# exoplanet-dev/exoplanet

Hardware: AMD Instinct MI355X
Metric: light-curve evals/sec (value+grad) at 150k cadences (higher is better)
Workload: dtype f64; 1 GPU; BASELINE configs[1] (C2): single planet e=0.3 Kepler solve + quadratic limb-darkened transit, 150000 cadences, value+grad, use_in_transit=False: dense flux output; n_cadences=150000, draws_per_gpu=1024, global_draws=1024, parallelism=draws sharded over 1 GPU(s); one collective of per-draw scalars per step

## Files before the change

### exoplanet_amd/_lib.py

```python
import ctypes
import os

_HERE = os.path.dirname(os.path.abspath(__file__))
LIB_PATH = os.environ.get("EXOPLANET_AMD_LIB") or os.path.join(_HERE, "lib", "libexoplanet_amd.so")
ABI_VERSION = 21

_c_dp = ctypes.c_void_p
_i64 = ctypes.c_int64
_i32 = ctypes.c_int32
_u32 = ctypes.c_uint32

_SIGNATURES = {
    "exo_abi_version": (_i32, []),
    "exo_kepler_f64": (ctypes.c_int, [_c_dp, _c_dp, _c_dp, _c_dp, _i64, _c_dp]),
    "exo_selftest_orbit_pos_f32": (ctypes.c_int, [_c_dp, _c_dp, _c_dp, _c_dp, _i64, _c_dp]),
    "exo_quad_solution_vector_f64": (ctypes.c_int, [_c_dp, _c_dp, _c_dp, _c_dp, _c_dp, _i64, _c_dp]),
    "exo_contact_points_f64": (ctypes.c_int, [_c_dp] * 10 + [_i64, _c_dp]),
    "exo_transit_flux_fwd_f64": (
        ctypes.c_int,
        [_c_dp, _i64, _c_dp, _i64, _c_dp, _c_dp, _i32, _c_dp, _c_dp, _i64, _i32, _u32, _c_dp, _c_dp, _i64, _c_dp],
    ),
    "exo_transit_flux_fwd_ev_f64": (
        ctypes.c_int,
        [_c_dp, _i64, _c_dp, _i64, _c_dp, _c_dp, _i32, _c_dp, _c_dp, _i64, _i32, _u32, _c_dp, _c_dp, _i64, _c_dp,
         _c_dp, _c_dp],
    ),
    "exo_transit_flux_workspace_bytes": (_i64, [_i64, _i64, _i32]),
    "exo_transit_flux_sparse_layout": (ctypes.c_int, [_i64, _i64, _i32, ctypes.POINTER(_i64)]),
    "exo_transit_flux_vjp_f64": (
        ctypes.c_int,
        [_c_dp, _i64, _c_dp, _i64, _c_dp, _c_dp, _i32, _c_dp, _c_dp, _i64, _i32, _u32,
         _c_dp, _c_dp, _c_dp, _c_dp, _c_dp, _c_dp, _i64, _c_dp],
    ),
    "exo_transit_flux_vjp_ev_f64": (
        ctypes.c_int,
        [_c_dp, _i64, _c_dp, _i64, _c_dp, _c_dp, _i32, _c_dp, _c_dp, _i64, _i32, _u32,
         _c_dp, _c_dp, _c_dp, _c_dp, _c_dp, _c_dp, _i64, _c_dp, _c_dp, _c_dp],
    ),
    "exo_transit_flux_ttv_fwd_f64": (
        ctypes.c_int,
        [_c_dp, _i64, _c_dp, _i64, _c_dp, _c_dp, _i32, _c_dp, _c_dp, _i64, _i32, _u32, _c_dp, _c_dp, _i32,
         _c_dp, _c_dp, _i64, _c_dp],
    ),
# ... 192 lines not shown
```

### exoplanet_amd/csrc/exo_transit.hip

```cpp
#include <hip/hip_runtime.h>
#include <stdint.h>

#include "../../include/exoplanet_amd.h"
#include "exo_contact.hpp"
#include "exo_math.hpp"
#include "exo_pack_core.hpp"
#include "exo_transit_list.hpp"
#include "exo_transit_merge.hpp"
#include "exo_transit_runs.hpp"
#include "exo_transit_sample.hpp"
#include "exo_transit_window.hpp"

namespace {

inline int launch_status() { return hipGetLastError() == hipSuccess ? EXO_OK : EXO_ERR_LAUNCH; }

struct Chi2Args {
  const double* obs;
  const double* ivar;
  int64_t n_ivar;
  double* chi2;
  const NoiseIn* nz = nullptr;
};

// ... 42 lines not shown
constexpr uint32_t kLikelihoodRefuses = EXO_FLAG_PER_PLANET | EXO_FLAG_SPARSE | EXO_FLAG_EXACT_SCAN;
constexpr uint32_t kTimedLikelihoodRefuses = kLikelihoodRefuses | EXO_FLAG_SECONDARY | EXO_FLAG_LIGHT_DELAY;
constexpr uint32_t kJacRefuses = EXO_FLAG_PER_PLANET | EXO_FLAG_EXACT_SCAN | EXO_FLAG_LIGHT_DELAY;
inline bool layout_ok(const Sweep& s) { return !((s.flags & EXO_FLAG_CADENCE_MAJOR) && (s.flags & EXO_FLAG_PER_PLANET)); }
inline bool exposure_ok(const Sweep& s) { return s.n_texp <= 0 || (s.texp && s.stencil_dt && s.stencil_w); }
inline bool ttv_ok(const Ttv& v, bool reverse) {
  return v.edges && v.shift && v.n_edge >= 1 && v.n_edge <= EXO_MAX_TTV_EDGES && (!reverse || v.gshift);
}
inline bool grad_ptrs_ok(const Sweep& s, const SweepOut& o) {
  return s.params && s.ld && o.gparams && o.gld && (s.n_cad <= 0 || s.t);
}
inline bool runs_path(const Sweep& s) {
  if (s.has_ttv() && (s.flags & (EXO_FLAG_SECONDARY | EXO_FLAG_LIGHT_DELAY))) return false;
  return s.n_texp <= 1 && !(s.flags & EXO_FLAG_EXACT_SCAN);
}
inline bool grad_slots_fit(const Sweep& s) { return s.n_planet * kNG + 7 <= kBlock; }
inline bool fit_runs(const void* workspace, int64_t workspace_bytes, int64_t n_cad, int64_t n_draw, int32_t n_planet, RunWs* rw) {
  *rw = carve_runs(const_cast<void*>(workspace), n_cad, n_draw, n_planet);
  return workspace && workspace_bytes >= rw->bytes;
}
inline bool fit_runs(const Sweep& s, RunWs* rw) { return fit_runs(s.workspace, s.workspace_bytes, s.n_cad, s.n_draw, s.n_planet, rw); }
inline int zero_grads(const Sweep& s, const SweepOut& o) {
  if (!exo::zero_fill_async(o.gparams, (int64_t)(s.n_draw * s.n_planet * EXO_NPAR), s.st)) return EXO_ERR_LAUNCH;
  if (o.flux_dot && !exo::zero_fill_async(o.flux_dot, (int64_t)(s.n_draw), s.st)) return EXO_ERR_LAUNCH;
  return exo::zero_fill_async(o.gld, (int64_t)(s.n_draw * (s.secondary() ? 6 : 3)), s.st) ? EXO_OK : EXO_ERR_LAUNCH;
}
inline bool zero_gshift(const Sweep& s) {
  return exo::zero_fill_async(s.ttv.gshift, (int64_t)(s.n_draw * s.n_planet * (s.ttv.n_edge + 1)), s.st);
}

template <bool G, bool SEC, bool LDELAY = false, bool CHI2 = false, bool TTV = false, bool JAC = false>
inline void launch_runs(const Sweep& s, const RunWs& w, const double* gflux, const double* gsparse, double* vals, int32_t* vcad,
                        double* fill, double* partial, const FinishArgs& fin, int64_t chi2_nw = 0) {
  hipLaunchKernelGGL((transit_runs_kernel<G, SEC, LDELAY, CHI2, TTV, JAC>), dim3((unsigned)w.hb, (unsigned)s.n_draw), dim3(kBlock), 0,
                     s.st, s.t, s.n_cad, s.texp, s.n_texp, s.stencil_dt, s.stencil_w, (int)s.n_sub, s.params, s.ld, (int)s.n_planet,
                     s.flags, s.n_ev(), w.rl, gflux, gsparse, vals, vcad, fill, partial, chi2_nw, s.ttv, fin);
}
template <bool G>
inline void launch_runs_plain(const Sweep& s, const RunWs& w, const double* gflux, const double* gsparse, double* vals,
                              int32_t* vcad, double* fill, double* partial, const FinishArgs& fin) {
  exo::with_flag(s.secondary(), [&](auto sec) {
    exo::with_flag(s.flags & EXO_FLAG_LIGHT_DELAY, [&](auto ldl) {
      launch_runs<G, decltype(sec)::value, decltype(ldl)::value>(s, w, gflux, gsparse, vals, vcad, fill, partial, fin);
    });
  });
}
inline int enumerate_runs(const Sweep& s, const SweepOut& o, const RunWs& w) {
  const bool fused = (s.flags & EXO_FLAG_SORTED_TIMES) && !s.has_ttv();
  if (o.pack && (!fused || o.reuse_runs)) return EXO_ERR_INVALID_ARGUMENT;
  const int n_ev = s.n_ev();
  const dim3 lists((unsigned)(s.n_draw * s.n_planet * n_ev)), wave(64);
// ... 39 lines not shown
                       s.n_cad, s.flags, s.n_ev(), w.rl, w.vcad, f.chi2_part, f.n_chi2_part, f.chi2, f.ttv, o.chi2->nz->out);
  else
    hipLaunchKernelGGL(transit_finish_kernel, grid, block, 0, s.st, f.partial, w.hb, (int)s.n_planet, s.secondary(), o.gparams, o.gld,
                       f.dot, s.n_cad, s.flags, s.n_ev(), w.rl, f.vals, w.vcad, f.fill, f.chi2_part, f.n_chi2_part, f.chi2, f.ttv);
  return launch_status();
}

inline bool single_pass(const Sweep& s) { return s.n_planet == 1 && !s.secondary() && s.n_sub == 1; }
inline int likelihood_single_pass(const Sweep& s, const SweepOut& o, const RunWs& w) {
  const Chi2Args& c = *o.chi2;
  const bool fold = own_block_finishes(s, o, w), ldelay = s.flags & EXO_FLAG_LIGHT_DELAY;
  const FinishArgs fin{o.gparams, o.gld, c.chi2, fold ? 1 : 0, w.done};
  const auto launch = [&](auto ldl, auto tv) {
    constexpr bool LDELAY = decltype(ldl)::value, TTV = decltype(tv)::value;
    if (c.nz)
      hipLaunchKernelGGL((transit_runs_kernel<true, false, LDELAY, true, TTV, false, true>), dim3((unsigned)w.hb, (unsigned)s.n_draw),
                         dim3(kBlock), 0, s.st, s.t, s.n_cad, s.texp, s.n_texp, s.stencil_dt, s.stencil_w, (int)s.n_sub, s.params, s.ld,
                         (int)s.n_planet, s.flags, s.n_ev(), w.rl, c.obs, c.ivar, nullptr, nullptr, nullptr, w.partial, c.n_ivar,
                         s.ttv, fin, *c.nz);
    else
      launch_runs<true, false, LDELAY, true, TTV>(s, w, c.obs, c.ivar, nullptr, nullptr, nullptr, w.partial, fin, c.n_ivar);
  };
  if (s.has_ttv()) launch(std::false_type{}, std::true_type{});
  else if (ldelay) launch(std::true_type{}, std::false_type{});
  else launch(std::false_type{}, std::false_type{});
  if (launch_status() != EXO_OK) return EXO_ERR_LAUNCH;
  if (fold) return EXO_OK;
  return launch_finish(s, o, w, FinishIn{w.partial, c.chi2, nullptr, nullptr, nullptr, 0, nullptr, s.ttv});
}

inline int likelihood_three_sweeps(const Sweep& s, const SweepOut& o, const RunWs& w) {
  const Chi2Args& c = *o.chi2;
  const FinishArgs no_fin{nullptr, nullptr, nullptr, 0, nullptr};
  const dim3 grid(kResidualBlocks, (unsigned)s.n_draw), block(kBlock);
// ... 56 lines not shown

int64_t exo_transit_flux_workspace_bytes(int64_t n_cad, int64_t n_draw, int32_t n_planet) {
  if (n_cad < 0 || n_draw < 0 || n_planet < 1) return -1;
  if (n_cad == 0 || n_draw == 0) return 0;
  int bpd, tpb;
  transit_geometry(n_cad, n_draw, &bpd, &tpb);
  const Workspace w = carve(nullptr, n_draw, bpd, tpb, n_planet);
  const RunWs r = carve_runs(nullptr, n_cad, n_draw, n_planet);
  return w.bytes > r.bytes ? w.bytes : r.bytes;
}

int exo_transit_flux_sparse_layout(int64_t n_cad, int64_t n_draw, int32_t n_planet, int64_t* out) {
  if (n_cad < 0 || n_draw < 0 || n_planet < 1 || !out) return EXO_ERR_INVALID_ARGUMENT;
  const RunWs r = carve_runs(nullptr, n_cad, n_draw, n_planet);
  out[0] = r.off_nrun; out[1] = r.off_runs; out[2] = r.off_pre_all; out[3] = r.off_vals; out[4] = r.rl.r_max;
  return EXO_OK;
}

int exo_transit_sparse_scatter_f64(const void* workspace, int64_t workspace_bytes, int64_t n_cad, int64_t n_draw, int32_t n_planet,
                                   uint32_t flags, int32_t clear, double* flux, void* stream) {
  if (!shape_ok(n_cad, n_draw, n_planet) || !draws_ok(n_draw) || (flags & ~(uint32_t)EXO_FLAG_SECONDARY))
    return EXO_ERR_INVALID_ARGUMENT;
  if (n_cad == 0 || n_draw == 0) return EXO_OK;
  if (!flux) return EXO_ERR_INVALID_ARGUMENT;
  RunWs rw;
  if (!fit_runs(workspace, workspace_bytes, n_cad, n_draw, n_planet, &rw)) return EXO_ERR_WORKSPACE;
  exo::with_flag(clear, [&](auto clr) {
    hipLaunchKernelGGL(transit_scatter_runs_kernel<decltype(clr)::value>, dim3((unsigned)n_draw), dim3(kBlock), 0, (hipStream_t)stream,
                       rw.rl, rw.vals, n_cad, (int)n_planet, events(flags), flux);
  });
// ... 419 lines not shown
```

### exoplanet_amd/csrc/exo_transit_runs.hpp

```cpp
#pragma once
#include "exo_pack_core.hpp"
#include "exo_transit_sample.hpp"
#include "exo_transit_window.hpp"

namespace {

struct Run {
  int32_t lo, a, b, hi;
};
constexpr int kRunMax = 4096;
#ifndef EXO_RUN_SEG
#define EXO_RUN_SEG 256
#endif
constexpr int kSeg = EXO_RUN_SEG;

struct RunLists {
  int32_t* nrun;
  Run* runs;
  int32_t* pre_in;
  int32_t* pre_all;
  int32_t* rbin;
  double* grun;
  int r_max;
};

__device__ __forceinline__ void enum_prefix(int (*s_len)[kRunMax + 1], int K, int lane, int32_t* __restrict__ pin,
                                            int32_t* __restrict__ pall, int32_t* __restrict__ nrun_dst) {
  const int per = (K + 63) / 64, k0 = lane * per, k1 = (k0 + per < K) ? k0 + per : K;
  int sum_in = 0, sum_all = 0;
// ... 253 lines not shown
        if (s_first[mid] <= r) lo_k = mid; else hi_k = mid;
      }
      const int k = lo_k;
      const double kc = (double)(s_mlo[k] + (r - s_first[k]));
      const double sh = row.shift[k];
      const auto guess = [&](double thr) { return ceil(((thr - c0) / nrev + sh - t_first) / t_rate); };
      const PhaseSearch ps{t, nrev, c0, -sh * nrev};
      ps.window_run(kc, h0, hin, (int)n_cad, t_rate > 0.0, guess, r, runs, s_len);
      rbin[r] = k;
    }
  }
  __syncthreads();
  enum_prefix(s_len, K, lane, pin, pall, rl.nrun + list);
}

struct FillCursor {
  typedef double v2d __attribute__((ext_vector_type(2)));
  char* base;
  int64_t off;
  int left;
  uint32_t loff;
  v2d zero;
  __device__ __forceinline__ FillCursor(double* dst, int64_t n) : base(nullptr), off(0), left(0), loff((threadIdx.x & 63) * 16) {
    zero = v2d{0.0, 0.0};
    asm volatile("" : "+v"(zero));
    if (!dst || n <= 0) return;
    const int64_t head = (reinterpret_cast<uintptr_t>(dst) & 8) ? 1 : 0;
    if (threadIdx.x == 0 && head) dst[0] = 0.0;
    if (threadIdx.x == 0 && ((n - head) & 1)) dst[n - 1] = 0.0;
    v2d* q2 = reinterpret_cast<v2d*>(dst + head);
    const int64_t n2 = (n - head) >> 1;
    const int64_t nfull = n2 >> 6;
    const int rem = (int)(n2 & 63);
    if ((int)threadIdx.x < rem) __builtin_nontemporal_store(zero, q2 + (nfull << 6) + threadIdx.x);
    const int w = __builtin_amdgcn_readfirstlane((int)(threadIdx.x >> 6));
    left = nfull > w ? (int)((nfull - w + kWaves - 1) / kWaves) : 0;
    left = __builtin_amdgcn_readfirstlane(left);
    base = reinterpret_cast<char*>(q2);
    off = (int64_t)w * 1024;
  }
  __device__ __forceinline__ int pieces_left() const { return left; }
  __device__ __forceinline__ void issue(int count) {
    const int k = count < left ? count : left;
    for (int s = 0; s < k; ++s) {
      __builtin_nontemporal_store(zero, reinterpret_cast<v2d*>(base + off + loff));
      off += kWaves * 1024;
    }
    left -= k;
  }
};

struct NoiseOut {
  double* gmean;
  double* gjit2;
};
template <bool NOISE = false>
__device__ __forceinline__ void finish_draw(
    int64_t draw, const double* partial, int nblk, int n_planet, bool secondary, double* __restrict__ gparams,
    double* __restrict__ gld, double* __restrict__ flux_dot, int64_t n_cad, uint32_t flags, int n_ev, const RunLists& rl,
    const double* vals, const int32_t* vcad, double* flux,
    const double* __restrict__ chi2_part, int n_chi2_part, double* __restrict__ chi2_out, const Ttv& ttv,
// ... 120 lines not shown
  double* gld;
  double* flux_dot;
  int fold;
  int32_t* done;
};
struct NoiseIn {
  const double* mean;
  const double* jit2;
  int64_t n_mean, n_jit;
  NoiseOut out;
};

#ifndef EXO_RUNS_MIN_WAVES
#define EXO_RUNS_MIN_WAVES 3
#endif
constexpr int kJac = 16;
__device__ __forceinline__ int jac_slot(int s) {
  return s < G_PAD ? s : (s == G_SINI ? 9 : (s >= kNG && s < kNG + 6 ? 10 + (s - kNG) : -1));
}
template <bool GRAD, bool SECONDARY, bool LDELAY = false, bool CHI2 = false, bool TTV = false, bool JAC = false, bool NOISE = false>
__global__ __launch_bounds__(kBlock, LDELAY ? 2 : EXO_RUNS_MIN_WAVES) void transit_runs_kernel(
    const double* __restrict__ t, int64_t n_cad, const double* __restrict__ texp, int64_t n_texp,
    const double* __restrict__ stencil_dt, const double* __restrict__ stencil_w, int n_sub,
    const double* __restrict__ params, const double* __restrict__ ld, int n_planet, uint32_t flags, int n_ev, RunLists rl,
    const double* __restrict__ gflux, const double* __restrict__ gsparse, double* __restrict__ vals,
    int32_t* __restrict__ vcad, double* __restrict__ fill, double* __restrict__ partial, int64_t chi2_nw = 0,
    Ttv ttv = Ttv{nullptr, nullptr, nullptr, 0}, FinishArgs fin = FinishArgs{nullptr, nullptr, nullptr, 0, nullptr},
    NoiseIn nz = NoiseIn{nullptr, nullptr, 0, 0, NoiseOut{nullptr, nullptr}}) {
  static_assert(!NOISE || (CHI2 && GRAD && !SECONDARY && !JAC), "the sampled-mean / jitter likelihood is a CHI2 sweep");
  __shared__ Shared sh;
  __shared__ Run s_run[kSeg];
  __shared__ int2 s_pre[kSeg + 1];
  __shared__ int s_all[kSeg + 1];
  __shared__ int s_bin[TTV ? kSeg : 1];
  __shared__ double s_shift[TTV ? kSeg : 1];
  __shared__ double s_grun[(TTV && GRAD) ? kWaves : 1][(TTV && GRAD) ? kSeg : 1];
  __shared__ int s_rounds[2 * EXO_MAX_PLANETS];
  __shared__ double lds_acc[kNG + 7][kBlock];
  const int64_t draw = blockIdx.y;
  const int hb = gridDim.x, bx = blockIdx.x;
  stage_constants(sh, params, ld, stencil_dt, stencil_w, n_sub, n_planet, draw, SECONDARY);
  const bool per_planet = flags & EXO_FLAG_PER_PLANET;
  const int n_lists = n_planet * n_ev;
  auto slice = [&](int K, int& k0, int& k1) {
    k0 = (int)((int64_t)K * bx / hb);
    k1 = (int)((int64_t)K * (bx + 1) / hb);
  };
  if ((int)threadIdx.x < n_lists) {
    const int64_t list = draw * n_lists + threadIdx.x;
    int k0, k1;
    slice(rl.nrun[list], k0, k1);
    const int32_t* pall = rl.pre_all + list * (rl.r_max + 1);
    int rounds = 0;
    for (int kb = k0; kb < k1; kb += kSeg) {
      const int ke = (kb + kSeg < k1) ? kb + kSeg : k1;
      rounds += (pall[ke] - pall[kb] + kBlock - 1) / kBlock;
    }
    s_rounds[threadIdx.x] = rounds;
  }
  __syncthreads();
  int total_rounds = 0;
  for (int l = 0; l < n_lists; ++l) total_rounds += s_rounds[l];
  const int64_t npl = per_planet ? n_planet : 1, n_fill = n_cad * npl;
  const int64_t f0 = n_fill * bx / hb, f1 = n_fill * (bx + 1) / hb;
  FillCursor fc(fill ? fill + draw * n_fill + f0 : nullptr, f1 - f0);
  const int per_round =
      __builtin_amdgcn_readfirstlane(total_rounds > 0 ? (fc.pieces_left() + total_rounds - 1) / total_rounds : 0);

  static_assert(!JAC || (GRAD && !LDELAY && !CHI2 && !TTV), "the Jacobian sweep is the plain value + gradient evaluation");
  const int ng_draw = n_planet * kNG + 7;
  double* __restrict__ pout = (GRAD && !JAC) ? partial + ((int64_t)draw * hb + bx) * ng_draw : nullptr;
  double* __restrict__ jac = JAC ? partial : nullptr;
  const GradAcc acc{GRAD ? &lds_acc[0][threadIdx.x] : nullptr};
  if (GRAD) {
#pragma unroll
    for (int s = 0; s < kNG + 7; ++s) lds_acc[s][threadIdx.x] = 0.0;
  }
  double cld[6];
#pragma unroll
  for (int k = 0; k < 6; ++k) cld[k] = uniform((SECONDARY || k < 3) ? sh.c[k] : 0.0);
  const double te = (n_texp == 0) ? 0.0 : texp[0];
  const double sdt0 = uniform(sh.sdt[0]), sw0 = uniform(sh.sw[0]);
  const double nz_mean = NOISE ? uniform(nz.mean[nz.n_mean == 1 ? 0 : draw]) : 0.0;
  const double nz_jit2 = (NOISE && nz.n_jit > 0) ? uniform(nz.jit2[nz.n_jit == 1 ? 0 : draw]) : 0.0;
  for (int p = 0; p < n_planet; ++p) {
    const PlanetS c(sh.pc[p]);
    if (GRAD && p > 0) {
#pragma unroll
      for (int s = 0; s < kNG; ++s) lds_acc[s][threadIdx.x] = 0.0;
    }
    int64_t vbase = (draw * n_planet + p) * n_cad;
    const TtvRow row(ttv, TTV ? draw * n_planet + p : 0);
    double* __restrict__ grow = (TTV && GRAD) ? ttv.gshift + (draw * n_planet + p) * (int64_t)(ttv.n_edge + 1) : nullptr;
    const TtvGrad tgrad{(GRAD && TTV) ? &lds_acc[0][threadIdx.x] : nullptr, grow, nullptr};
    for (int ev = 0; ev < n_ev; ++ev) {
      const int64_t list = (draw * n_planet + p) * n_ev + ev;
      const int K = rl.nrun[list];
      const Run* __restrict__ runs = rl.runs + list * rl.r_max;
      const int32_t* __restrict__ pin = rl.pre_in + list * (rl.r_max + 1);
      const int32_t* __restrict__ pall = rl.pre_all + list * (rl.r_max + 1);
      int k0, k1;
      slice(K, k0, k1);
      for (int kb = k0; kb < k1; kb += kSeg) {
        const int m = (kb + kSeg < k1) ? kSeg : k1 - kb;
        __syncthreads();
        const int in0 = pin[kb], all0 = pall[kb];
        for (int q = threadIdx.x; q <= m; q += kBlock) {
          const int pi = pin[kb + q] - in0, pa = pall[kb + q];
          s_pre[q] = make_int2(pi, (pa - all0) - pi);
          s_all[q] = pa;
          if (q < m) s_run[q] = runs[kb + q];
          if (TTV && q < m) {
            const int kq = rl.rbin[list * rl.r_max + kb + q];
            s_bin[q] = kq;
            s_shift[q] = kq >= 0 ? row.shift[kq] : 0.0;
            if (GRAD) {
#pragma unroll
              for (int w = 0; w < kWaves; ++w) s_grun[w][q] = 0.0;
            }
          }
        }
        __syncthreads();
        const bool trusted = TTV && s_bin[0] >= 0;
        const int tin = s_pre[m].x, total = tin + s_pre[m].y;
        const float g_in = tin > 0 ? (float)m / (float)tin : 0.0f;
        const float g_lim = total > tin ? (float)m / (float)(total - tin) : 0.0f;
        struct Item { int i, v, q; double tv, g, w; };
        auto locate = [&](int j, int& i, int& v, int& qrun) {
          const bool in = j < tin;
          const int jj = in ? j : j - tin;
          int q = (int)((float)jj * (in ? g_in : g_lim));
          q = q < m - 1 ? q : m - 1;
          int2 pa = s_pre[q], pb = s_pre[q + 1];
          int lo = in ? pa.x : pa.y, hi = in ? pb.x : pb.y;
          int tries = 0;
          while (EXO_WAVE_ANY((jj < lo) | (jj >= hi))) {
            if (++tries > 4) {
              q = 0;
#pragma unroll
              for (int step = kSeg / 2; step > 0; step >>= 1) {
                const int c2 = q + step;
                if (c2 < m) {
                  const int2 pc = s_pre[c2];
                  q = (jj >= (in ? pc.x : pc.y)) ? c2 : q;
                }
              }
              pa = s_pre[q];
              lo = in ? pa.x : pa.y;
              break;
            }
            q += (jj < lo) ? -1 : ((jj >= hi) ? 1 : 0);
            pa = s_pre[q]; pb = s_pre[q + 1];
            lo = in ? pa.x : pa.y; hi = in ? pb.x : pb.y;
          }
          const Run r = s_run[q];
// ... 11 lines not shown
          } else if (NOISE) {
            if (j < total) {
              it.g = gflux[it.i] - nz_mean;
              it.w = exo::fast_rcp(gsparse[chi2_nw == 1 ? 0 : it.i] + nz_jit2);
            }
          } else if (CHI2) {
            if (j < total) { it.g = gflux[it.i]; it.w = gsparse[chi2_nw == 1 ? 0 : it.i]; }
          } else if (GRAD && j < total)
            it.g = gsparse ? gsparse[vbase + it.v]
                           : (per_planet ? gflux[(draw * n_cad + it.i) * n_planet + p]
                                         : ((flags & EXO_FLAG_CADENCE_MAJOR) ? gflux[(int64_t)it.i * gridDim.y + draw]
                                                                             : gflux[draw * n_cad + it.i]));
          return it;
        };
        Item nxt = load_item(threadIdx.x);
        for (int j0 = 0; j0 < total; j0 += kBlock) {
          const int j = j0 + threadIdx.x;
          const bool has = j < total;
          const Item cur = nxt;
          if (j0 + kBlock < total) nxt = load_item(j + kBlock);
          fc.issue(per_round);
          double f = 0.0;
          const double dsh = TTV ? s_shift[TTV ? cur.q : 0] : 0.0;
          for (int k = 0; k < n_sub; ++k) {
            const double sdt_k = (k == 0) ? sdt0 : sh.sdt[k], sw_k = (k == 0) ? sw0 : sh.sw[k];
            double tt = fma(te, sdt_k, cur.tv);
            int ks = 0;
            if (TTV) {
              double sh_k = dsh;
              if (!trusted) {
                ks = row.bin(tt);
                sh_k = row.shift[ks];
              }
              tt -= sh_k;
            }
            const double gw = cur.g * sw_k;
            const double F = eval_sample<GRAD, SECONDARY, LDELAY, CHI2>(tt, c, cld, CHI2 ? cur.g : gw, acc, cur.w);
            f = fma(sw_k, F, f);
            if (CHI2) {
              const double r = F - cur.g;
              acc.add(kNG + 6, cur.w * (r * r - cur.g * cur.g));
              if (NOISE) {
                acc.add(kNG + 3, cur.w * F);
                acc.add(kNG + 4, cur.w * cur.w * (r * r - cur.g * cur.g));
              }
            } else if (GRAD && !JAC) {
              acc.add(kNG + 6, gw * F);
            }
            if (TTV && GRAD && !trusted) tgrad.flush_lane(ks);
          }
          if (TTV && GRAD && trusted) tgrad.flush_runs(cur.q, &s_grun[0][0], kSeg);
          if (JAC) {
            double row[kJac];
#pragma unroll
            for (int q = 0; q < kJac; ++q) row[q] = 0.0;
#pragma unroll
            for (int sl = 0; sl < kNG + 6; ++sl) {
              if (jac_slot(sl) >= 0) {
                row[jac_slot(sl)] = lds_acc[sl][threadIdx.x];
                lds_acc[sl][threadIdx.x] = 0.0;
              }
            }
            if (has) {
              double2* __restrict__ dst = reinterpret_cast<double2*>(jac + (vbase + cur.v) * kJac);
#pragma unroll
              for (int q = 0; q < kJac / 2; ++q) dst[q] = make_double2(row[2 * q], row[2 * q + 1]);
            }
          }
          if (vals && has) {
            vals[vbase + cur.v] = f;
            if (vcad) vcad[vbase + cur.v] = cur.i;
          }
        }
        if (TTV && GRAD && trusted) {
          __syncthreads();
          for (int q = threadIdx.x; q < m; q += kBlock) {
            double v = s_grun[0][q];
#pragma unroll
            for (int w = 1; w < kWaves; ++w) v += s_grun[(TTV && GRAD) ? w : 0][q];
            rl.grun[list * rl.r_max + kb + q] = v;
          }
        }
      }
      vbase += pall[K];
    }
    if (GRAD && TTV) {
      lds_acc[G_TP][threadIdx.x] = lds_acc[G_PAD][threadIdx.x];
      lds_acc[G_PAD][threadIdx.x] = 0.0;
    }
    if (GRAD && !JAC) reduce_columns(lds_acc, sh.red, 0, kNG, pout + p * kNG);
  }
  if (GRAD && !JAC) reduce_columns(lds_acc, sh.red, kNG, 7, pout + n_planet * kNG);
  fc.issue(1 << 30);
  if (fin.fold) {
// ... 169 lines not shown
        }
      }
      const int tot = pall[K];
      vbase += (tot < 0 || tot > n_cad) ? 0 : tot;
    }
    if (!CLEAR && p + 1 < n_planet) __syncthreads();
  }
}

#ifndef EXO_RUNS_TARGET_BLOCKS
#define EXO_RUNS_TARGET_BLOCKS 512
#endif
inline int runs_blocks_per_draw(int64_t n_draw) {
  int64_t hb = (EXO_RUNS_TARGET_BLOCKS + n_draw - 1) / n_draw;
  return (int)(hb < 1 ? 1 : (hb > 64 ? 64 : hb));
}
inline int runs_r_max(int64_t n_cad) { return (int)(n_cad < kRunMax ? (n_cad < 16 ? 16 : n_cad) : kRunMax); }

struct RunWs {
  double* partial;
  double* windows;
  int32_t* sorted;
  RunLists rl;
  double* vals;
  int32_t* vcad;
  double* gvals;
  double* chi2_part;
  int32_t* done;
  int hb, n_sorted;
  int64_t off_nrun, off_runs, off_pre_all, off_vals;
// ... 31 lines not shown
```

### exoplanet_amd/csrc/exo_transit_sample.hpp

```cpp
#pragma once
#include <hip/hip_runtime.h>
#include <stdint.h>

#include "../../include/exoplanet_amd.h"
#include "exo_math.hpp"

namespace {

constexpr int kBlock = 256;
constexpr int kWaves = kBlock / 64;
constexpr int kTile = 2 * kBlock;
constexpr int kNG = 12;
constexpr int kWin = 7;
enum { G_N = 0, G_TP, G_ECC, G_COSW, G_SINW, G_COSI, G_AOR, G_ROR, G_FR, G_PAD, G_SINI, G_CL };
constexpr double kCLight = 37231.66360672704;

struct PlanetConst {
  double n, tp, e, se, pe, sq1me2, cw, sw, ci, si, aor, ror, iror;
  double t0, period, iperiod, ts, te, fr, ts2, te2, isq1me2;
  double clr;
  float ef, omf, sqf, cwf, swf, cif, zsf, thrf, zthrf, inthrf;
  double nrev, c0, dmid, half[2];
  double te0, tinv;
  int tfin;
// ... 134 lines not shown
__device__ __forceinline__ double uniform(double x) {
  const int lo = __builtin_amdgcn_readfirstlane(__double2loint(x));
  const int hi = __builtin_amdgcn_readfirstlane(__double2hiint(x));
  return __hiloint2double(hi, lo);
}

struct PlanetS {
  double n, tp, e, se, pe, sq1me2, isq1me2, cw, sw, ci, si, aor, ror, iror, fr, clr;
  __device__ __forceinline__ explicit PlanetS(const PlanetConst& c)
      : n(uniform(c.n)), tp(uniform(c.tp)), e(uniform(c.e)), se(uniform(c.se)), pe(uniform(c.pe)),
        sq1me2(uniform(c.sq1me2)), isq1me2(uniform(c.isq1me2)), cw(uniform(c.cw)), sw(uniform(c.sw)),
        ci(uniform(c.ci)), si(uniform(c.si)), aor(uniform(c.aor)), ror(uniform(c.ror)), iror(uniform(c.iror)),
        fr(uniform(c.fr)), clr(uniform(c.clr)) {}
};

struct GradAcc {
  double* col;
  __device__ __forceinline__ void add(int slot, double v) const {
    __hip_atomic_fetch_add(col + slot * kBlock, v, __ATOMIC_RELAXED, __HIP_MEMORY_SCOPE_WAVEFRONT);
  }
};

template <bool GRAD, bool SECONDARY, bool LDELAY = false, bool CHI2 = false>
__device__ __forceinline__ double eval_sample(double tt, const PlanetS& c, const double* cld,
                                              double gw, const GradAcc& acc, double c2w = 0.0) {
  double ld_cx = 0, ld_sx = 0, ld_den = 0, ld_z = 0, ld_vz = 0, ld_az = 0, ld_w = 0, ld_s = 0, ld_D = 0, ld_sig = 1, ld_t = tt;
  if (LDELAY) {
    const exo::KeplerHalf k1 = exo::kepler_half(exo::mean_anomaly_reduced(tt, c.tp, c.n), c.e, c.se, c.pe);
    const double X2 = k1.X * k1.X, Y2 = k1.Y * k1.Y;
    ld_cx = X2 - Y2; ld_sx = 2.0 * k1.X * k1.Y; ld_den = X2 + Y2;
    const double y1 = -c.aor * (c.sw * ld_cx + c.cw * ld_sx);
    ld_z = -c.si * y1;
    const double iden = exo::fast_div(1.0, ld_den);
    const double cwf = (c.cw * ld_cx - c.sw * ld_sx) * iden;
    ld_vz = -c.n * c.aor * c.isq1me2 * c.si * (c.e * c.cw + cwf);
    ld_az = -c.n * c.n * ld_z * iden * iden * iden;
    ld_sig = (SECONDARY && ld_z < 0.0) ? -1.0 : 1.0;
    const double q = -ld_sig * ld_z, ic = exo::fast_div(1.0, c.clr);
    ld_w = fma(ld_sig * ld_vz, ic, 1.0);
    ld_s = sqrt(fma(-2.0 * ld_sig * ld_az * q, ic * ic, ld_w * ld_w));
// ... 144 lines not shown
__device__ __forceinline__ double wave_sum_last(double v) {
  v = dpp_add<0x111, 0xf>(v);
  v = dpp_add<0x112, 0xf>(v);
  v = dpp_add<0x114, 0xf>(v);
  v = dpp_add<0x118, 0xf>(v);
  v = dpp_add<0x142, 0xa>(v);
  v = dpp_add<0x143, 0xc>(v);
  return v;
}

constexpr int kBinSlots = 16;
struct BinCache {
  double sum[kWaves][kBinSlots];
  int id[kWaves][kBinSlots];
};
struct TtvGrad {
  double* __restrict__ col;
  double* __restrict__ grow;
  BinCache* cache;
  __device__ __forceinline__ double take() const {
    const double d = col[G_TP * kBlock];
    col[G_TP * kBlock] = 0.0;
    col[G_PAD * kBlock] += d;
    return d;
  }
  __device__ __forceinline__ void flush_lane(int k) const {
    const double d = take();
    if (d != 0.0) unsafeAtomicAdd(grow + k, d);
  }
  __device__ __forceinline__ void flush_wave(int k) const {
    const double d = take();
    unsigned long long todo = __ballot(d != 0.0);
    while (todo) {
      const int first = __builtin_amdgcn_readfirstlane(__ffsll((long long)todo) - 1);
      const int k0 = __builtin_amdgcn_readlane(k, first);
      const bool mine = k == k0;
      const double sum = wave_sum_last(mine ? d : 0.0);
      todo &= ~__ballot(mine);
// ... 22 lines not shown
      todo &= ~__ballot(mine);
      const int w = __builtin_amdgcn_readfirstlane((int)(threadIdx.x >> 6));
      if ((threadIdx.x & 63) == 63) tab[w * row_len + q0] += sum;
    }
  }
  __device__ __forceinline__ void drain() const {
    __syncthreads();
    if (threadIdx.x < kWaves * kBinSlots) {
      const int k = (&cache->id[0][0])[threadIdx.x];
      if (k >= 0) unsafeAtomicAdd(grow + k, (&cache->sum[0][0])[threadIdx.x]);
      (&cache->id[0][0])[threadIdx.x] = -1;
    }
    __syncthreads();
  }
};

__device__ __forceinline__ void reduce_columns(double (*acc)[kBlock], double (*red)[16], int first, int n,
    double* __restrict__ out) {
  __syncthreads();
  const int s = threadIdx.x >> 4, c = threadIdx.x & 15;
  if (s < n) {
    double v = 0.0;
#pragma unroll
    for (int i = 0; i < kBlock / 16; ++i) v += acc[first + s][c + 16 * i];
    red[s][c] = v;
  }
  __syncthreads();
  if ((int)threadIdx.x < n) {
    double v = 0.0;
#pragma unroll
    for (int i = 0; i < 16; ++i) v += red[threadIdx.x][i];
    out[threadIdx.x] = v;
  }
  __syncthreads();
}

template <class Extra>
__device__ __forceinline__ void partials_to_gradients(int64_t draw, const double* partial, int nblk, int n_planet,
                                                      bool secondary, int nthr, double* gparams, double* gld,
// ... 37 lines not shown
```

### exoplanet_amd/ops.py

```python
import ctypes
import os
import warnings
from types import SimpleNamespace
from typing import NamedTuple, Optional

import numpy as np
import torch

from . import _lib

NPAR = 20
(P_N, P_TP, P_ECC, P_COSW, P_SINW, P_COSI, P_SINI, P_AOR, P_ROR, P_T0, P_PERIOD, P_TS, P_TE,
 P_FRATIO, P_TS2, P_TE2, P_CLIGHT) = range(17)
FLAG_PER_PLANET = 1
FLAG_WINDOW = 2
FLAG_SECONDARY = 4
PACK_CIRCULAR = 8
FLAG_EXACT_SCAN = 16
FLAG_SPARSE = 32
FLAG_LIGHT_DELAY = 64
FLAG_CADENCE_MAJOR = 128
FLAG_SORTED_TIMES = 256
NIN = 10
(IN_PERIOD, IN_T0, IN_B, IN_ECC, IN_OMEGA, IN_R, IN_MSTAR, IN_RSTAR, IN_MPLANET, IN_SBR) = range(10)
# ... 116 lines not shown


def _workspace(N, D, P, device, zero=False):
    nbytes = _workspace_bytes(N, D, P)
    return (torch.zeros if zero else torch.empty)(max(nbytes // 8 + 1, 1), dtype=torch.float64, device=device), nbytes


def _layout(name, N, D, P):
    lay = (ctypes.c_int64 * 5)()
    _call(name, None, N, D, P, lay)
    return list(lay)


def _sparse_layout(N, D, P):
    return _layout("exo_transit_flux_sparse_layout", N, D, P)


def _merge_layout(N, D, P):
    return _layout("exo_sparse_merge_layout", N, D, P)


def is_cadence_major(x):
    return (torch.is_tensor(x) and x.is_cuda and x.dtype == torch.float64 and x.dim() == 2 and x.shape[0] > 1
            and x.stride() == (1, x.shape[0]))


class _Kepler(torch.autograd.Function):
    @staticmethod
    def forward(ctx, M, ecc):
        M = _dev(M, "M")
# ... 1724 lines not shown
```

### include/exoplanet_amd.h

```cpp
#ifndef EXOPLANET_AMD_H
#define EXOPLANET_AMD_H

#include <stdint.h>

#ifdef __cplusplus
extern "C" {
#endif

#define EXO_OK 0
#define EXO_ERR_INVALID_ARGUMENT 1
#define EXO_ERR_LAUNCH 2
#define EXO_ERR_WORKSPACE 3

#define EXO_ABI_VERSION 21
int32_t exo_abi_version(void);

int exo_kepler_f64(const double* M, const double* ecc, double* sinf, double* cosf,
                   int64_t n, void* stream);

int exo_quad_solution_vector_f64(const double* b, const double* r, double* s,
                                 double* dsdb, double* dsdr, int64_t n, void* stream);

int exo_contact_points_f64(const double* a, const double* e, const double* cosw,
                           const double* sinw, const double* cosi, const double* sini,
// ... 35 lines not shown
#define EXO_FLAG_SWEEP_ALL (EXO_FLAG_PER_PLANET | EXO_FLAG_WINDOW | EXO_FLAG_SECONDARY | EXO_FLAG_EXACT_SCAN | \
                            EXO_FLAG_SPARSE | EXO_FLAG_LIGHT_DELAY | EXO_FLAG_CADENCE_MAJOR | EXO_FLAG_SORTED_TIMES)

#define EXO_MAX_PLANETS 16
#define EXO_MAX_SUBEXP 63

int exo_transit_flux_fwd_f64(const double* t, int64_t n_cad, const double* texp, int64_t n_texp,
                             const double* stencil_dt, const double* stencil_w, int32_t n_sub,
                             const double* params, const double* ld, int64_t n_draw,
                             int32_t n_planet, uint32_t flags, double* flux, void* workspace,
                             int64_t workspace_bytes, void* stream);

int64_t exo_transit_flux_workspace_bytes(int64_t n_cad, int64_t n_draw, int32_t n_planet);

int exo_transit_flux_sparse_layout(int64_t n_cad, int64_t n_draw, int32_t n_planet, int64_t* out);

typedef struct exo_sparse_model {
  const int32_t* nseg;
  const int32_t* seg;
  const int32_t* off;
  const double* vals;
  int64_t seg_row, off_row, val_row;
  int32_t seg_step, hi_at;
  const int32_t* row_of_draw;
} exo_sparse_model;
int exo_transit_flux_sparse_model(const void* workspace, int64_t workspace_bytes, int64_t n_cad, int64_t n_draw,
                                  int32_t n_planet, uint32_t flags, exo_sparse_model* out);
int64_t exo_sparse_merge_workspace_bytes(int64_t n_cad, int64_t n_draw, int32_t n_planet);
int exo_sparse_merge_layout(int64_t n_cad, int64_t n_draw, int32_t n_planet, int64_t* out);
int exo_sparse_model_merge_f64(const void* workspace, int64_t workspace_bytes, int64_t n_cad, int64_t n_draw, int32_t n_planet,
// ... 374 lines not shown
```

Baseline: 3.686 million evals/s.

## Pick a 192- or 256-thread block for the runs kernel per device and grid

```diff
diff --git a/exoplanet_amd/_lib.py b/exoplanet_amd/_lib.py
--- a/exoplanet_amd/_lib.py
+++ b/exoplanet_amd/_lib.py
@@ -27,6 +27,7 @@
     ),
     "exo_transit_flux_workspace_bytes": (_i64, [_i64, _i64, _i32]),
     "exo_transit_flux_sparse_layout": (ctypes.c_int, [_i64, _i64, _i32, ctypes.POINTER(_i64)]),
+    "exo_transit_runs_geometry": (ctypes.c_int, [_i64, _i32, ctypes.POINTER(_i32), ctypes.POINTER(_i32)]),
     "exo_transit_flux_vjp_f64": (
         ctypes.c_int,
         [_c_dp, _i64, _c_dp, _i64, _c_dp, _c_dp, _i32, _c_dp, _c_dp, _i64, _i32, _u32,
diff --git a/exoplanet_amd/csrc/exo_transit.hip b/exoplanet_amd/csrc/exo_transit.hip
--- a/exoplanet_amd/csrc/exo_transit.hip
+++ b/exoplanet_amd/csrc/exo_transit.hip
@@ -1,5 +1,8 @@
 #include <hip/hip_runtime.h>
 #include <stdint.h>
+
+#include <atomic>
+#include <type_traits>
 
 #include "../../include/exoplanet_amd.h"
 #include "exo_contact.hpp"
@@ -80,7 +83,23 @@
   if (s.has_ttv() && (s.flags & (EXO_FLAG_SECONDARY | EXO_FLAG_LIGHT_DELAY))) return false;
   return s.n_texp <= 1 && !(s.flags & EXO_FLAG_EXACT_SCAN);
 }
-inline bool grad_slots_fit(const Sweep& s) { return s.n_planet * kNG + 7 <= kBlock; }
+inline bool grad_slots_fit(const Sweep& s, int threads = kBlock) { return s.n_planet * kNG + 7 <= threads; }
+inline int device_cus() {
+  constexpr int kMaxDev = 64;
+  static std::atomic<int> cus[kMaxDev];
+  int dev = 0;
+  if (hipGetDevice(&dev) != hipSuccess || dev < 0 || dev >= kMaxDev) return 0;
+  int n = cus[dev].load(std::memory_order_relaxed);
+  if (n == 0) {
+    if (hipDeviceGetAttribute(&n, hipDeviceAttributeMultiprocessorCount, dev) != hipSuccess || n < 1) return 0;
+    cus[dev].store(n, std::memory_order_relaxed);
+  }
+  return n;
+}
+inline int runs_block_threads(const Sweep& s, const RunWs& w, bool has_narrow, bool fills) {
+  const bool narrow_ok = has_narrow && (!fills || EXO_RUNS_BLOCK_WAVES == 3) && grad_slots_fit(s, kBlockNarrow);
+  return 64 * runs_block_waves(s.n_draw * w.hb, narrow_ok ? device_cus() : 0, narrow_ok);
+}
 inline bool fit_runs(const void* workspace, int64_t workspace_bytes, int64_t n_cad, int64_t n_draw, int32_t n_planet, RunWs* rw) {
   *rw = carve_runs(const_cast<void*>(workspace), n_cad, n_draw, n_planet);
   return workspace && workspace_bytes >= rw->bytes;
@@ -95,12 +114,20 @@
   return exo::zero_fill_async(s.ttv.gshift, (int64_t)(s.n_draw * s.n_planet * (s.ttv.n_edge + 1)), s.st);
 }
 
-template <bool G, bool SEC, bool LDELAY = false, bool CHI2 = false, bool TTV = false, bool JAC = false>
+template <bool G, bool SEC, bool LDELAY = false, bool CHI2 = false, bool TTV = false, bool JAC = false, bool NOISE = false>
 inline void launch_runs(const Sweep& s, const RunWs& w, const double* gflux, const double* gsparse, double* vals, int32_t* vcad,
-                        double* fill, double* partial, const FinishArgs& fin, int64_t chi2_nw = 0) {
-  hipLaunchKernelGGL((transit_runs_kernel<G, SEC, LDELAY, CHI2, TTV, JAC>), dim3((unsigned)w.hb, (unsigned)s.n_draw), dim3(kBlock), 0,
-                     s.st, s.t, s.n_cad, s.texp, s.n_texp, s.stencil_dt, s.stencil_w, (int)s.n_sub, s.params, s.ld, (int)s.n_planet,
-                     s.flags, s.n_ev(), w.rl, gflux, gsparse, vals, vcad, fill, partial, chi2_nw, s.ttv, fin);
+                        double* fill, double* partial, const FinishArgs& fin, int64_t chi2_nw = 0,
+                        const NoiseIn& nz = NoiseIn{nullptr, nullptr, 0, 0, NoiseOut{nullptr, nullptr}}) {
+  const auto launch = [&](auto bw) {
+    constexpr int BW = decltype(bw)::value;
+    hipLaunchKernelGGL((transit_runs_kernel<G, SEC, LDELAY, CHI2, TTV, JAC, NOISE, BW>), dim3((unsigned)w.hb, (unsigned)s.n_draw),
+                       dim3(BW), 0, s.st, s.t, s.n_cad, s.texp, s.n_texp, s.stencil_dt, s.stencil_w, (int)s.n_sub, s.params, s.ld,
+                       (int)s.n_planet, s.flags, s.n_ev(), w.rl, gflux, gsparse, vals, vcad, fill, partial, chi2_nw, s.ttv, fin, nz);
+  };
+  if constexpr (runs_has_narrow(LDELAY, TTV)) {
+    if (runs_block_threads(s, w, true, fill != nullptr) == kBlockNarrow) return launch(std::integral_constant<int, kBlockNarrow>{});
+  }
+  launch(std::integral_constant<int, kBlock>{});
 }
 template <bool G>
 inline void launch_runs_plain(const Sweep& s, const RunWs& w, const double* gflux, const double* gsparse, double* vals,
@@ -170,10 +197,8 @@
   const auto launch = [&](auto ldl, auto tv) {
     constexpr bool LDELAY = decltype(ldl)::value, TTV = decltype(tv)::value;
     if (c.nz)
-      hipLaunchKernelGGL((transit_runs_kernel<true, false, LDELAY, true, TTV, false, true>), dim3((unsigned)w.hb, (unsigned)s.n_draw),
-                         dim3(kBlock), 0, s.st, s.t, s.n_cad, s.texp, s.n_texp, s.stencil_dt, s.stencil_w, (int)s.n_sub, s.params, s.ld,
-                         (int)s.n_planet, s.flags, s.n_ev(), w.rl, c.obs, c.ivar, nullptr, nullptr, nullptr, w.partial, c.n_ivar,
-                         s.ttv, fin, *c.nz);
+      launch_runs<true, false, LDELAY, true, TTV, false, true>(s, w, c.obs, c.ivar, nullptr, nullptr, nullptr, w.partial, fin, c.n_ivar,
+                                                               *c.nz);
     else
       launch_runs<true, false, LDELAY, true, TTV>(s, w, c.obs, c.ivar, nullptr, nullptr, nullptr, w.partial, fin, c.n_ivar);
   };
@@ -260,6 +285,15 @@
   if (n_cad < 0 || n_draw < 0 || n_planet < 1 || !out) return EXO_ERR_INVALID_ARGUMENT;
   const RunWs r = carve_runs(nullptr, n_cad, n_draw, n_planet);
   out[0] = r.off_nrun; out[1] = r.off_runs; out[2] = r.off_pre_all; out[3] = r.off_vals; out[4] = r.rl.r_max;
+  return EXO_OK;
+}
+
+int exo_transit_runs_geometry(int64_t n_draw, int32_t n_cu, int32_t* blocks_per_draw, int32_t* block_threads) {
+  if (n_draw < 1 || !blocks_per_draw || !block_threads) return EXO_ERR_INVALID_ARGUMENT;
+  const int hb = runs_blocks_per_draw(n_draw);
+  const int cus = n_cu > 0 ? n_cu : device_cus();
+  *blocks_per_draw = hb;
+  *block_threads = 64 * runs_block_waves(n_draw * hb, cus, runs_has_narrow(false, false));
   return EXO_OK;
 }
 
diff --git a/exoplanet_amd/csrc/exo_transit_runs.hpp b/exoplanet_amd/csrc/exo_transit_runs.hpp
--- a/exoplanet_amd/csrc/exo_transit_runs.hpp
+++ b/exoplanet_amd/csrc/exo_transit_runs.hpp
@@ -13,6 +13,9 @@
 #define EXO_RUN_SEG 256
 #endif
 constexpr int kSeg = EXO_RUN_SEG;
+constexpr int kBlockNarrow = 192;
+constexpr int kSegNarrow = kSeg < 128 ? kSeg : 128;
+constexpr int runs_seg(int bw) { return bw == kBlock ? kSeg : kSegNarrow; }
 
 struct RunLists {
   int32_t* nrun;
@@ -296,6 +299,7 @@
   enum_prefix(s_len, K, lane, pin, pall, rl.nrun + list);
 }
 
+template <int WAVES>
 struct FillCursor {
   typedef double v2d __attribute__((ext_vector_type(2)));
   char* base;
@@ -316,7 +320,7 @@
     const int rem = (int)(n2 & 63);
     if ((int)threadIdx.x < rem) __builtin_nontemporal_store(zero, q2 + (nfull << 6) + threadIdx.x);
     const int w = __builtin_amdgcn_readfirstlane((int)(threadIdx.x >> 6));
-    left = nfull > w ? (int)((nfull - w + kWaves - 1) / kWaves) : 0;
+    left = nfull > w ? (int)((nfull - w + WAVES - 1) / WAVES) : 0;
     left = __builtin_amdgcn_readfirstlane(left);
     base = reinterpret_cast<char*>(q2);
     off = (int64_t)w * 1024;
@@ -326,7 +330,7 @@
     const int k = count < left ? count : left;
     for (int s = 0; s < k; ++s) {
       __builtin_nontemporal_store(zero, reinterpret_cast<v2d*>(base + off + loff));
-      off += kWaves * 1024;
+      off += WAVES * 1024;
     }
     left -= k;
   }
@@ -477,12 +481,14 @@
 #ifndef EXO_RUNS_MIN_WAVES
 #define EXO_RUNS_MIN_WAVES 3
 #endif
+constexpr bool runs_has_narrow(bool ldelay, bool ttv) { return !ldelay && !ttv && EXO_RUNS_MIN_WAVES == 3; }
 constexpr int kJac = 16;
 __device__ __forceinline__ int jac_slot(int s) {
   return s < G_PAD ? s : (s == G_SINI ? 9 : (s >= kNG && s < kNG + 6 ? 10 + (s - kNG) : -1));
 }
-template <bool GRAD, bool SECONDARY, bool LDELAY = false, bool CHI2 = false, bool TTV = false, bool JAC = false, bool NOISE = false>
-__global__ __launch_bounds__(kBlock, LDELAY ? 2 : EXO_RUNS_MIN_WAVES) void transit_runs_kernel(
+template <bool GRAD, bool SECONDARY, bool LDELAY = false, bool CHI2 = false, bool TTV = false, bool JAC = false, bool NOISE = false,
+          int BW = kBlock>
+__global__ __launch_bounds__(BW, LDELAY ? 2 : EXO_RUNS_MIN_WAVES) void transit_runs_kernel(
     const double* __restrict__ t, int64_t n_cad, const double* __restrict__ texp, int64_t n_texp,
     const double* __restrict__ stencil_dt, const double* __restrict__ stencil_w, int n_sub,
     const double* __restrict__ params, const double* __restrict__ ld, int n_planet, uint32_t flags, int n_ev, RunLists rl,
@@ -491,15 +497,17 @@
     Ttv ttv = Ttv{nullptr, nullptr, nullptr, 0}, FinishArgs fin = FinishArgs{nullptr, nullptr, nullptr, 0, nullptr},
     NoiseIn nz = NoiseIn{nullptr, nullptr, 0, 0, NoiseOut{nullptr, nullptr}}) {
   static_assert(!NOISE || (CHI2 && GRAD && !SECONDARY && !JAC), "the sampled-mean / jitter likelihood is a CHI2 sweep");
+  static_assert(BW == kBlock || (BW == kBlockNarrow && runs_has_narrow(LDELAY, TTV)), "256 threads, or 192 at three waves per SIMD");
+  constexpr int kWavesB = BW / 64, kSegB = runs_seg(BW);
   __shared__ Shared sh;
-  __shared__ Run s_run[kSeg];
-  __shared__ int2 s_pre[kSeg + 1];
-  __shared__ int s_all[kSeg + 1];
-  __shared__ int s_bin[TTV ? kSeg : 1];
-  __shared__ double s_shift[TTV ? kSeg : 1];
-  __shared__ double s_grun[(TTV && GRAD) ? kWaves : 1][(TTV && GRAD) ? kSeg : 1];
+  __shared__ Run s_run[kSegB];
+  __shared__ int2 s_pre[kSegB + 1];
+  __shared__ int s_all[kSegB + 1];
+  __shared__ int s_bin[TTV ? kSegB : 1];
+  __shared__ double s_shift[TTV ? kSegB : 1];
+  __shared__ double s_grun[(TTV && GRAD) ? kWavesB : 1][(TTV && GRAD) ? kSegB : 1];
   __shared__ int s_rounds[2 * EXO_MAX_PLANETS];
-  __shared__ double lds_acc[kNG + 7][kBlock];
+  __shared__ double lds_acc[kNG + 7][BW];
   const int64_t draw = blockIdx.y;
   const int hb = gridDim.x, bx = blockIdx.x;
   stage_constants(sh, params, ld, stencil_dt, stencil_w, n_sub, n_planet, draw, SECONDARY);
@@ -515,9 +523,9 @@
     slice(rl.nrun[list], k0, k1);
     const int32_t* pall = rl.pre_all + list * (rl.r_max + 1);
     int rounds = 0;
-    for (int kb = k0; kb < k1; kb += kSeg) {
-      const int ke = (kb + kSeg < k1) ? kb + kSeg : k1;
-      rounds += (pall[ke] - pall[kb] + kBlock - 1) / kBlock;
+    for (int kb = k0; kb < k1; kb += kSegB) {
+      const int ke = (kb + kSegB < k1) ? kb + kSegB : k1;
+      rounds += (pall[ke] - pall[kb] + BW - 1) / BW;
     }
     s_rounds[threadIdx.x] = rounds;
   }
@@ -526,7 +534,7 @@
   for (int l = 0; l < n_lists; ++l) total_rounds += s_rounds[l];
   const int64_t npl = per_planet ? n_planet : 1, n_fill = n_cad * npl;
   const int64_t f0 = n_fill * bx / hb, f1 = n_fill * (bx + 1) / hb;
-  FillCursor fc(fill ? fill + draw * n_fill + f0 : nullptr, f1 - f0);
+  FillCursor<kWavesB> fc(fill ? fill + draw * n_fill + f0 : nullptr, f1 - f0);
   const int per_round =
       __builtin_amdgcn_readfirstlane(total_rounds > 0 ? (fc.pieces_left() + total_rounds - 1) / total_rounds : 0);
 
@@ -534,7 +542,7 @@
   const int ng_draw = n_planet * kNG + 7;
   double* __restrict__ pout = (GRAD && !JAC) ? partial + ((int64_t)draw * hb + bx) * ng_draw : nullptr;
   double* __restrict__ jac = JAC ? partial : nullptr;
-  const GradAcc acc{GRAD ? &lds_acc[0][threadIdx.x] : nullptr};
+  const GradAccT<BW> acc{GRAD ? &lds_acc[0][threadIdx.x] : nullptr};
   if (GRAD) {
 #pragma unroll
     for (int s = 0; s < kNG + 7; ++s) lds_acc[s][threadIdx.x] = 0.0;
@@ -555,7 +563,7 @@
     int64_t vbase = (draw * n_planet + p) * n_cad;
     const TtvRow row(ttv, TTV ? draw * n_planet + p : 0);
     double* __restrict__ grow = (TTV && GRAD) ? ttv.gshift + (draw * n_planet + p) * (int64_t)(ttv.n_edge + 1) : nullptr;
-    const TtvGrad tgrad{(GRAD && TTV) ? &lds_acc[0][threadIdx.x] : nullptr, grow, nullptr};
+    const TtvGradT<BW> tgrad{(GRAD && TTV) ? &lds_acc[0][threadIdx.x] : nullptr, grow, nullptr};
     for (int ev = 0; ev < n_ev; ++ev) {
       const int64_t list = (draw * n_planet + p) * n_ev + ev;
       const int K = rl.nrun[list];
@@ -564,11 +572,11 @@
       const int32_t* __restrict__ pall = rl.pre_all + list * (rl.r_max + 1);
       int k0, k1;
       slice(K, k0, k1);
-      for (int kb = k0; kb < k1; kb += kSeg) {
-        const int m = (kb + kSeg < k1) ? kSeg : k1 - kb;
+      for (int kb = k0; kb < k1; kb += kSegB) {
+        const int m = (kb + kSegB < k1) ? kSegB : k1 - kb;
         __syncthreads();
         const int in0 = pin[kb], all0 = pall[kb];
-        for (int q = threadIdx.x; q <= m; q += kBlock) {
+        for (int q = threadIdx.x; q <= m; q += BW) {
           const int pi = pin[kb + q] - in0, pa = pall[kb + q];
           s_pre[q] = make_int2(pi, (pa - all0) - pi);
           s_all[q] = pa;
@@ -579,7 +587,7 @@
             s_shift[q] = kq >= 0 ? row.shift[kq] : 0.0;
             if (GRAD) {
 #pragma unroll
-              for (int w = 0; w < kWaves; ++w) s_grun[w][q] = 0.0;
+              for (int w = 0; w < kWavesB; ++w) s_grun[w][q] = 0.0;
             }
           }
         }
@@ -601,7 +609,7 @@
             if (++tries > 4) {
               q = 0;
 #pragma unroll
-              for (int step = kSeg / 2; step > 0; step >>= 1) {
+              for (int step = kSegB / 2; step > 0; step >>= 1) {
                 const int c2 = q + step;
                 if (c2 < m) {
                   const int2 pc = s_pre[c2];
@@ -643,11 +651,11 @@
           return it;
         };
         Item nxt = load_item(threadIdx.x);
-        for (int j0 = 0; j0 < total; j0 += kBlock) {
+        for (int j0 = 0; j0 < total; j0 += BW) {
           const int j = j0 + threadIdx.x;
           const bool has = j < total;
           const Item cur = nxt;
-          if (j0 + kBlock < total) nxt = load_item(j + kBlock);
+          if (j0 + BW < total) nxt = load_item(j + BW);
           fc.issue(per_round);
           double f = 0.0;
           const double dsh = TTV ? s_shift[TTV ? cur.q : 0] : 0.0;
@@ -678,7 +686,7 @@
             }
             if (TTV && GRAD && !trusted) tgrad.flush_lane(ks);
           }
-          if (TTV && GRAD && trusted) tgrad.flush_runs(cur.q, &s_grun[0][0], kSeg);
+          if (TTV && GRAD && trusted) tgrad.flush_runs(cur.q, &s_grun[0][0], kSegB);
           if (JAC) {
             double row[kJac];
 #pragma unroll
@@ -703,10 +711,10 @@
         }
         if (TTV && GRAD && trusted) {
           __syncthreads();
-          for (int q = threadIdx.x; q < m; q += kBlock) {
+          for (int q = threadIdx.x; q < m; q += BW) {
             double v = s_grun[0][q];
 #pragma unroll
-            for (int w = 1; w < kWaves; ++w) v += s_grun[(TTV && GRAD) ? w : 0][q];
+            for (int w = 1; w < kWavesB; ++w) v += s_grun[(TTV && GRAD) ? w : 0][q];
             rl.grun[list * rl.r_max + kb + q] = v;
           }
         }
@@ -906,6 +914,17 @@
 inline int runs_blocks_per_draw(int64_t n_draw) {
   int64_t hb = (EXO_RUNS_TARGET_BLOCKS + n_draw - 1) / n_draw;
   return (int)(hb < 1 ? 1 : (hb > 64 ? 64 : hb));
+}
+#ifndef EXO_RUNS_BLOCK_WAVES
+#define EXO_RUNS_BLOCK_WAVES 0
+#endif
+static_assert(EXO_RUNS_BLOCK_WAVES == 0 || EXO_RUNS_BLOCK_WAVES == 3 || EXO_RUNS_BLOCK_WAVES == 4, "0 (the rule), 3 or 4");
+inline int runs_block_waves(int64_t n_blocks, int n_cu, bool narrow_ok) {
+  if (!narrow_ok || EXO_RUNS_BLOCK_WAVES == 4 || n_cu < 1) return 4;
+  if (EXO_RUNS_BLOCK_WAVES == 3) return 3;
+  const int64_t slots3 = (int64_t)n_cu * 4, slots4 = (int64_t)n_cu * 3;
+  const int64_t gen3 = (n_blocks + slots3 - 1) / slots3, gen4 = (n_blocks + slots4 - 1) / slots4;
+  return gen3 * 4 < gen4 * 3 ? 3 : 4;
 }
 inline int runs_r_max(int64_t n_cad) { return (int)(n_cad < kRunMax ? (n_cad < 16 ? 16 : n_cad) : kRunMax); }
 
diff --git a/exoplanet_amd/csrc/exo_transit_sample.hpp b/exoplanet_amd/csrc/exo_transit_sample.hpp
--- a/exoplanet_amd/csrc/exo_transit_sample.hpp
+++ b/exoplanet_amd/csrc/exo_transit_sample.hpp
@@ -172,16 +172,18 @@
         fr(uniform(c.fr)), clr(uniform(c.clr)) {}
 };
 
-struct GradAcc {
+template <int BW = kBlock>
+struct GradAccT {
   double* col;
   __device__ __forceinline__ void add(int slot, double v) const {
-    __hip_atomic_fetch_add(col + slot * kBlock, v, __ATOMIC_RELAXED, __HIP_MEMORY_SCOPE_WAVEFRONT);
-  }
-};
-
-template <bool GRAD, bool SECONDARY, bool LDELAY = false, bool CHI2 = false>
+    __hip_atomic_fetch_add(col + slot * BW, v, __ATOMIC_RELAXED, __HIP_MEMORY_SCOPE_WAVEFRONT);
+  }
+};
+using GradAcc = GradAccT<>;
+
+template <bool GRAD, bool SECONDARY, bool LDELAY = false, bool CHI2 = false, class Acc = GradAcc>
 __device__ __forceinline__ double eval_sample(double tt, const PlanetS& c, const double* cld,
-                                              double gw, const GradAcc& acc, double c2w = 0.0) {
+                                              double gw, const Acc& acc, double c2w = 0.0) {
   double ld_cx = 0, ld_sx = 0, ld_den = 0, ld_z = 0, ld_vz = 0, ld_az = 0, ld_w = 0, ld_s = 0, ld_D = 0, ld_sig = 1, ld_t = tt;
   if (LDELAY) {
     const exo::KeplerHalf k1 = exo::kepler_half(exo::mean_anomaly_reduced(tt, c.tp, c.n), c.e, c.se, c.pe);
@@ -356,14 +358,15 @@
   double sum[kWaves][kBinSlots];
   int id[kWaves][kBinSlots];
 };
-struct TtvGrad {
+template <int BW = kBlock>
+struct TtvGradT {
   double* __restrict__ col;
   double* __restrict__ grow;
   BinCache* cache;
   __device__ __forceinline__ double take() const {
-    const double d = col[G_TP * kBlock];
-    col[G_TP * kBlock] = 0.0;
-    col[G_PAD * kBlock] += d;
+    const double d = col[G_TP * BW];
+    col[G_TP * BW] = 0.0;
+    col[G_PAD * BW] += d;
     return d;
   }
   __device__ __forceinline__ void flush_lane(int k) const {
@@ -416,15 +419,18 @@
     __syncthreads();
   }
 };
-
-__device__ __forceinline__ void reduce_columns(double (*acc)[kBlock], double (*red)[16], int first, int n,
+using TtvGrad = TtvGradT<>;
+
+template <int BW>
+__device__ __forceinline__ void reduce_columns(double (*acc)[BW], double (*red)[16], int first, int n,
     double* __restrict__ out) {
+  static_assert(BW % 64 == 0 && BW / 16 >= kNG, "a thread per (slot, column mod 16) for up to kNG slots");
   __syncthreads();
   const int s = threadIdx.x >> 4, c = threadIdx.x & 15;
   if (s < n) {
     double v = 0.0;
 #pragma unroll
-    for (int i = 0; i < kBlock / 16; ++i) v += acc[first + s][c + 16 * i];
+    for (int i = 0; i < BW / 16; ++i) v += acc[first + s][c + 16 * i];
     red[s][c] = v;
   }
   __syncthreads();
diff --git a/exoplanet_amd/ops.py b/exoplanet_amd/ops.py
--- a/exoplanet_amd/ops.py
+++ b/exoplanet_amd/ops.py
@@ -154,6 +154,12 @@
 
 def _sparse_layout(N, D, P):
     return _layout("exo_transit_flux_sparse_layout", N, D, P)
+
+
+def transit_runs_geometry(n_draw, n_cu=0):
+    hb, threads = ctypes.c_int32(), ctypes.c_int32()
+    _call("exo_transit_runs_geometry", None, int(n_draw), int(n_cu), ctypes.byref(hb), ctypes.byref(threads))
+    return hb.value, threads.value
 
 
 def _merge_layout(N, D, P):
diff --git a/include/exoplanet_amd.h b/include/exoplanet_amd.h
--- a/include/exoplanet_amd.h
+++ b/include/exoplanet_amd.h
@@ -73,6 +73,8 @@
 int64_t exo_transit_flux_workspace_bytes(int64_t n_cad, int64_t n_draw, int32_t n_planet);
 
 int exo_transit_flux_sparse_layout(int64_t n_cad, int64_t n_draw, int32_t n_planet, int64_t* out);
+
+int exo_transit_runs_geometry(int64_t n_draw, int32_t n_cu, int32_t* blocks_per_draw, int32_t* block_threads);
 
 typedef struct exo_sparse_model {
   const int32_t* nseg;
```

Result: slower. 3.568 million evals/s (-3.2%).
